# HBioquant/DiffBindFR

Hardware: AMD Instinct MI355X
Metric: poses_per_sec (higher is better)
Workload: dtype f32

## Files before the change

diffbindfr_amd/csrc/convz.hip:

```cpp
#include <cstdio>
#include <cstdlib>
#include <type_traits>

#include "common.h"

typedef float f32x4 __attribute__((ext_vector_type(4)));
typedef float f32x2 __attribute__((ext_vector_type(2)));
typedef _Float16 f16x8 __attribute__((ext_vector_type(8)));
typedef _Float16 f16x4 __attribute__((ext_vector_type(4)));
typedef _Float16 f16x2 __attribute__((ext_vector_type(2)));
typedef unsigned u32x4 __attribute__((ext_vector_type(4)));
typedef unsigned u32x2 __attribute__((ext_vector_type(2)));

#define CH_TILE_BYTES 9280
#define CH_TAIL_OFF 8192
#define CH_BIAS_OFF 9216

#define CZ_VSTRIDE 2064
#define CZ_CB (8 * CZ_VSTRIDE)
#define CZ_NCB 2
#define CZ_TILE (CZ_NCB * CZ_CB)
#define CZ_KPB 1
#define CZ_BUF (CZ_KPB * CZ_TILE)
#define CZ_ZBYTES (2 * CZ_BUF)
#define CZ_WAVE_FLOATS (32 * 12 + 32 + 32 + 32 + 32 + 32 + CZ_MAXSEG * 16 + 24 * 64)
#ifndef CZ_PRIO
#define CZ_PRIO 1
#endif
#if CZ_PRIO
#define CZ_SETPRIO(x) __builtin_amdgcn_s_setprio(x)
#else
#define CZ_SETPRIO(x)
#endif
#ifndef CZ_FETCH_AT
#define CZ_FETCH_AT 4
#endif
#ifndef CZ_PF_KT
#define CZ_PF_KT 7
#endif
#define CZ_ZSCALE (-20)

__device__ __forceinline__ void cz_split2(float x0, float x1, unsigned& hi, unsigned& lo) {
  const f16x2 h = __builtin_convertvector((f32x2){x0, x1}, f16x2);
  const f16x2 l = __builtin_convertvector((f32x2){x0 - (float)h[0], x1 - (float)h[1]}, f16x2);
  hi = __builtin_bit_cast(unsigned, h);
  lo = __builtin_bit_cast(unsigned, l);
}
__device__ __forceinline__ float cz_wave_max(float v) {
#pragma unroll
  for (int o = 1; o < 64; o <<= 1) v = fmaxf(v, __shfl_xor(v, o));
  return v;
}

template <int I, int N, typename F>
__device__ __forceinline__ void cz_static_for(F&& f) {
  if constexpr (I < N) { f(std::integral_constant<int, I>{}); cz_static_for<I + 1, N>(f); }
}

template <int NW, int ABL = 0>
__global__ __launch_bounds__(64 * NW, 2) void k_convz(ConvZArgs a) {
  constexpr int KT = 9;
  extern __shared__ __attribute__((aligned(16))) float lds[];
  const int tid = threadIdx.x, lane = tid & 63, wave = __builtin_amdgcn_readfirstlane(tid >> 6);
  const int n = lane & 15, g = lane >> 4;
  char* zb = reinterpret_cast<char*>(lds);
  float* wl = lds + CZ_ZBYTES / 4 + wave * CZ_WAVE_FLOATS;
  float* w_sh = wl;
  float* w_sa = wl + 32 * 12;
  float* w_ua = w_sa + 32;
  int* w_row = reinterpret_cast<int*>(w_ua + 32);
  int* w_seg = w_row + 32;
  int* w_first = w_seg + 32;
  unsigned* w_mask = reinterpret_cast<unsigned*>(w_first + 32);
  float* w_xs = reinterpret_cast<float*>(w_mask + CZ_MAXSEG * 16);
  int* b_nseg = reinterpret_cast<int*>(lds + CZ_ZBYTES / 4 + NW * CZ_WAVE_FLOATS);
  int* b_col_edge = b_nseg + NW;
  float* b_col_inv = reinterpret_cast<float*>(b_col_edge + 16 * CZ_NCB);
  unsigned* b_cdesc = reinterpret_cast<unsigned*>(b_col_inv + 16 * CZ_NCB);

  int tr_n = 0;
  auto stamp = [&](int tag) {
    if constexpr ((ABL & 128) != 0) {
      if (a.dbg && blockIdx.x == 0 && lane == 0 && tr_n < 1000) {
        unsigned long long* t = reinterpret_cast<unsigned long long*>(a.dbg) + wave * 1024;
        t[tr_n++] = (__builtin_amdgcn_s_memtime() << 8) | (unsigned)tag;
      }
    }
  };
  int nch[4] = {0, 0, 0, 0}, nu[4] = {0, 0, 0, 0};
#pragma unroll
  for (int c = 0; c < 4; ++c)
    if (c < a.n_conv) {
      const ConvZDesc& d = a.c[c];
      nch[c] = min(*d.n_chunks, d.max_chunks);
      nu[c] = (nch[c] + NW - 1) / NW;
    }
  const int N = nu[0] + nu[1] + nu[2] + nu[3];
  for (int unit = blockIdx.x; unit < N; unit += gridDim.x) {
    int c = 0, ul = unit;
    if (ul >= nu[0]) { ul -= nu[0]; c = 1; if (ul >= nu[1]) { ul -= nu[1]; c = 2; if (ul >= nu[2]) { ul -= nu[2]; c = 3; } } }
    const ConvZDesc& d = a.c[c];
    const ConvZ& W = d.w;
    const int E = min(*d.n_edges, d.max_edges);
    const int ch = ul * NW + wave;
    int es = 0, len = 0, gidx = 0;
    if (ch < nch[c]) {
      es = d.chunk_es[ch];
      const int gl = d.chunk_gl[ch];
      gidx = gl >> 6;
      len = min(min(gl & 63, 32), max(E - es, 0));
    }
    __syncthreads();
    if (tid < CZ_MAXCT * 16) b_cdesc[tid] = tid < (W.ct0[W.n_io - 1] + W.nct[W.n_io - 1]) * 16 ? W.cdesc[tid] : 0u;
    if (unit != (int)blockIdx.x) tr_n = 1000;
    stamp(1);
    const int sl = lane & 31;
    const bool have = len > 0;
    const int e_sl = have ? es + min(sl, len - 1) : 0;
    int tgt_l = 0, gth_l = 0;
    if (have) { tgt_l = d.tgt[e_sl]; gth_l = d.gth[e_sl]; }
    const int tgt_prev = __shfl_up(tgt_l, 1);
    const bool is_first = lane < 32 && sl < len && (sl == 0 || tgt_l != tgt_prev);
    const unsigned long long bal = __ballot(is_first);
    const unsigned firsts = (unsigned)bal;
    const int nseg = min(__popc(firsts), CZ_MAXSEG);
    const int seg_l = (sl < len) ? __popc(firsts & (0xffffffffu >> (31 - sl))) - 1 : -1;
    if (lane < 32) {
      w_row[sl] = gth_l * d.ldx;
      w_seg[sl] = seg_l;
      if (is_first) w_first[seg_l] = sl;
      const float* sp = d.sh + (size_t)e_sl * SH_LD;
#pragma unroll
      for (int k = 0; k < 9; ++k) w_sh[sl * 12 + k] = have ? sp[k] : 0.f;
      w_sh[sl * 12 + 9] = w_sh[sl * 12 + 10] = w_sh[sl * 12 + 11] = 0.f;
    }
    if (lane == 0) b_nseg[wave] = nseg;
    float xmx = 0.f, smx = 0.f;
    if (have) {
      if (d.xmax) xmx = d.xmax[gidx];
      else {
        const float* xr = d.x + (size_t)gth_l * d.ldx;
        const int d4 = d.ldx >> 2;
        for (int j = lane >> 5; j < d4; j += 2) {
          const f32x4 v = *reinterpret_cast<const f32x4*>(xr + 4 * j);
          xmx = fmaxf(fmaxf(xmx, fmaxf(fabsf(v[0]), fabsf(v[1]))), fmaxf(fabsf(v[2]), fabsf(v[3])));
        }
      }
      if (lane < 32) {
        const float* sp = d.sh + (size_t)e_sl * SH_LD;
#pragma unroll
        for (int k = 0; k < 9; ++k) smx = fmaxf(smx, fabsf(sp[k]));
      }
    }
    xmx = cz_wave_max(xmx); smx = cz_wave_max(smx);
    int ey = 0;
    if (xmx > 0.f && smx > 0.f) ey = max(-100, min(100, 13 - __builtin_amdgcn_frexp_expf(xmx) - __builtin_amdgcn_frexp_expf(smx)));
    ey = __builtin_amdgcn_readfirstlane(ey);
    const float sY = __builtin_amdgcn_ldexpf(1.f, ey);

    stamp(2);
    u32x4 Hh[CZ_NKT][2];
    int eh = 0;
    {
      const __amdgpu_buffer_rsrc_t rW1 = __builtin_amdgcn_make_buffer_rsrc((void*)W.W1h, 0, KT * CH_TILE_BYTES, 0x00020000);
      u32x4 Ah[2][2][4];
      u32x4 Atc[2];
#pragma unroll
      for (int et = 0; et < 2; ++et) {
        const int slot = 16 * et + n;
        const int e = have ? es + min(slot, len - 1) : 0;
        const float* r0 = d.emb + (size_t)e * NS;
        const float* r1 = d.tab1 + (size_t)(have ? d.idx1[e] : 0) * d.ld1;
        const float* r2 = d.tab2 + (size_t)(have ? d.idx2[e] : 0) * d.ld2;
        f32x4 Ba[KT];
        float amx = 0.f;
#pragma unroll
        for (int s4 = 0; s4 < KT; ++s4) {
          const float* src = s4 < 3 ? r0 : s4 < 6 ? r1 : r2;
          Ba[s4] = have ? *reinterpret_cast<const f32x4*>(src + 16 * (s4 % 3) + 4 * g) : (f32x4){0.f, 0.f, 0.f, 0.f};
#pragma unroll
          for (int q = 0; q < 4; ++q) amx = fmaxf(amx, fabsf(Ba[s4][q]));
        }
        amx = fmaxf(amx, __shfl_xor(amx, 16));
        amx = fmaxf(amx, __shfl_xor(amx, 32));
        const int ja = max(-14, __builtin_amdgcn_frexp_expf(amx));
        const float sa = __builtin_amdgcn_ldexpf(1.f, 15 - ja);
        if (g == 0) { w_sa[slot] = sa; w_ua[slot] = __builtin_amdgcn_ldexpf(1.f, ja - 15); }
#pragma unroll
        for (int s4 = 0; s4 < KT; ++s4) {
          unsigned hi0, lo0, hi1, lo1;
          cz_split2(Ba[s4][0] * sa, Ba[s4][1] * sa, hi0, lo0);
          cz_split2(Ba[s4][2] * sa, Ba[s4][3] * sa, hi1, lo1);
          if (s4 < 8) {
            Ah[et][0][s4 >> 1][2 * (s4 & 1)] = hi0; Ah[et][0][s4 >> 1][2 * (s4 & 1) + 1] = hi1;
            Ah[et][1][s4 >> 1][2 * (s4 & 1)] = lo0; Ah[et][1][s4 >> 1][2 * (s4 & 1) + 1] = lo1;
          } else {
            Atc[et] = (u32x4){lo0, lo1, hi0, hi1};
          }
        }
      }
      __builtin_amdgcn_wave_barrier();
      f32x4 sar[2], uar[2];
#pragma unroll
      for (int et = 0; et < 2; ++et) {
        sar[et] = *reinterpret_cast<const f32x4*>(w_sa + 16 * et + 4 * g);
        uar[et] = *reinterpret_cast<const f32x4*>(w_ua + 16 * et + 4 * g);
      }
      float Hf[KT][2][4];
      float hmx = 0.f;
      const int vW = lane * 16;
      u32x4 F[3][2];
      auto ldF = [&](auto ic) {
        constexpr int i = decltype(ic)::value, m = i / 5, sx = i % 5;
        if constexpr (sx < 4) {
          F[i % 3][0] = __builtin_bit_cast(u32x4, __builtin_amdgcn_raw_buffer_load_b128(rW1, vW, m * CH_TILE_BYTES + sx * 1024, 0));
          F[i % 3][1] = __builtin_bit_cast(u32x4, __builtin_amdgcn_raw_buffer_load_b128(rW1, vW, m * CH_TILE_BYTES + (4 + sx) * 1024, 0));
        } else {
          F[i % 3][0] = __builtin_bit_cast(u32x4, __builtin_amdgcn_raw_buffer_load_b128(rW1, vW, m * CH_TILE_BYTES + CH_TAIL_OFF, 0));
          F[i % 3][1][0] = __builtin_amdgcn_raw_buffer_load_b32(rW1, n * 4, m * CH_TILE_BYTES + CH_BIAS_OFF, 0);
        }
      };
      ldF(std::integral_constant<int, 0>{});
      ldF(std::integral_constant<int, 1>{});
      f32x4 acc[2];
      cz_static_for<0, 5 * KT>([&](auto ic) {
        constexpr int i = decltype(ic)::value, m = i / 5, sx = i % 5;
        if constexpr (i + 2 < 5 * KT) ldF(std::integral_constant<int, (i + 2 < 5 * KT ? i + 2 : 0)>{});
        if constexpr (sx == 0) { acc[0] = (f32x4){0.f, 0.f, 0.f, 0.f}; acc[1] = (f32x4){0.f, 0.f, 0.f, 0.f}; }
        if constexpr (sx < 4) {
          const f16x8 whi = __builtin_bit_cast(f16x8, F[i % 3][0]), wlo = __builtin_bit_cast(f16x8, F[i % 3][1]);
#pragma unroll
          for (int et = 0; et < 2; ++et) {
            acc[et] = __builtin_amdgcn_mfma_f32_16x16x32_f16(__builtin_bit_cast(f16x8, Ah[et][1][sx]), whi, acc[et], 0, 0, 0);
            acc[et] = __builtin_amdgcn_mfma_f32_16x16x32_f16(__builtin_bit_cast(f16x8, Ah[et][0][sx]), wlo, acc[et], 0, 0, 0);
            acc[et] = __builtin_amdgcn_mfma_f32_16x16x32_f16(__builtin_bit_cast(f16x8, Ah[et][0][sx]), whi, acc[et], 0, 0, 0);
          }
        } else {
          const u32x4 wt = F[i % 3][0];
          const f16x8 wf = __builtin_bit_cast(f16x8, wt);
          const f16x8 wh = __builtin_bit_cast(f16x8, (u32x4){wt[0], wt[1], 0u, 0u});
          const float bias = __builtin_bit_cast(float, F[i % 3][1][0]);
          const float w1r = W.W1rinv ? W.W1rinv[16 * m + n] : 1.f;
#pragma unroll
          for (int et = 0; et < 2; ++et) {
            acc[et] = __builtin_amdgcn_mfma_f32_16x16x32_f16(__builtin_bit_cast(f16x8, Atc[et]), wf, acc[et], 0, 0, 0);
            acc[et] = __builtin_amdgcn_mfma_f32_16x16x32_f16(__builtin_bit_cast(f16x8, (u32x4){Atc[et][2], Atc[et][3], 0u, 0u}), wh, acc[et], 0, 0, 0);
          }
#pragma unroll
          for (int et = 0; et < 2; ++et)
#pragma unroll
            for (int q = 0; q < 4; ++q) {
              const float v = fmaxf(acc[et][q] + bias * sar[et][q], 0.f) * (uar[et][q] * w1r);
              Hf[m][et][q] = v;
              hmx = fmaxf(hmx, v);
            }
        }
      });
      if (!(ABL & 128) && a.dbg && unit == 0 && wave == 0) {
        const float k1i = __builtin_amdgcn_ldexpf(1.f, -W.k1);
#pragma unroll
        for (int m = 0; m < KT; ++m)
#pragma unroll
          for (int et = 0; et < 2; ++et)
#pragma unroll
            for (int q = 0; q < 4; ++q) a.dbg[(16 * et + 4 * g + q) * 144 + 16 * m + n] = Hf[m][et][q] * k1i;
      }
      hmx = cz_wave_max(hmx);
      eh = max(hmx > 0.f ? __builtin_amdgcn_frexp_expf(hmx) : W.k1, W.k1);
      eh = min(eh, W.k1 + 100);
      const float sH = __builtin_amdgcn_ldexpf(1.f, 15 - eh);
#pragma unroll
      for (int m = 0; m < KT; ++m) {
        unsigned h0, l0, h1, l1, h2, l2, h3, l3;
        cz_split2(Hf[m][0][0] * sH, Hf[m][0][1] * sH, h0, l0);
        cz_split2(Hf[m][0][2] * sH, Hf[m][0][3] * sH, h1, l1);
        cz_split2(Hf[m][1][0] * sH, Hf[m][1][1] * sH, h2, l2);
        cz_split2(Hf[m][1][2] * sH, Hf[m][1][3] * sH, h3, l3);
        Hh[m][0] = (u32x4){h0, h1, h2, h3};
        Hh[m][1] = (u32x4){l0, l1, l2, l3};
      }
    }
    const int ephi = 15 - eh + W.k1;
    {
      const _Float16 ph = (_Float16)__builtin_amdgcn_ldexpf(1.f, ephi);
      const unsigned short pb = __builtin_bit_cast(unsigned short, ph);
      u32x4 hb = {0u, 0u, 0u, 0u};
      if (n == 0) {
#pragma unroll
        for (int t = 0; t < 8; ++t) {
          const int slot = t < 4 ? 4 * g + t : 16 + 4 * g + (t - 4);
          if (slot < len) hb[t >> 1] |= (unsigned)pb << (16 * (t & 1));
        }
      }
      Hh[KT][0] = hb;
      Hh[KT][1] = (u32x4){0u, 0u, 0u, 0u};
    }
    stamp(3);
    {
      const int j = lane >> 4, gg = (lane >> 2) & 3, r = lane & 3, t0 = 2 * r;
      const int s0 = t0 < 4 ? 4 * gg + t0 : 16 + 4 * gg + (t0 - 4);
      w_mask[lane] = (w_seg[s0] == j ? 0x0000ffffu : 0u) | (w_seg[s0 + 1] == j ? 0xffff0000u : 0u);
    }
    __builtin_amdgcn_wave_barrier();
    __syncthreads();
    int cbase = 0, total = 0;
#pragma unroll
    for (int v = 0; v < NW; ++v) { const int c = b_nseg[v]; if (v < wave) cbase += c; total += c; }
    cbase = __builtin_amdgcn_readfirstlane(cbase); total = __builtin_amdgcn_readfirstlane(total);
    const int nseg_u = __builtin_amdgcn_readfirstlane(nseg);
    const int ncb = (total + 15) >> 4;
    const float col_inv = __builtin_amdgcn_ldexpf(1.f, -CZ_ZSCALE - ey - ephi);
    const float zs = __builtin_amdgcn_ldexpf(1.f, CZ_ZSCALE);
    if (ABL & 32) continue;
    for (int c = tid; c < 16 * CZ_NCB; c += 64 * NW) b_col_edge[c] = -1;
    __syncthreads();
    if (lane < nseg_u) {
      b_col_edge[cbase + lane] = es + w_first[lane];
      b_col_inv[cbase + lane] = col_inv;
    }
    char* za[CZ_MAXSEG];
    {
      char* zw0 = zb + (n & 7) * CZ_VSTRIDE + g * 512 + (n >> 3) * 256;
#pragma unroll
      for (int j = 0; j < CZ_MAXSEG; ++j) {
        const int col = cbase + j;
        za[j] = j < nseg_u ? zw0 + (col >> 4) * CZ_CB + (col & 15) * 16 : zw0 + CZ_CB + 15 * 16;
      }
    }
    long long n_mfma = 2 * KT * 14;
    for (int io = 0; io < W.n_io; ++io) {
      n_mfma += (long long)W.nct[io] * (3LL * CZ_NKT * CZ_MAXSEG + 9LL * ncb * (KT + (wave == 0)));
      f32x4 acc[3][CZ_NCB];
#pragma unroll
      for (int wt = 0; wt < 3; ++wt)
#pragma unroll
        for (int cb = 0; cb < CZ_NCB; ++cb) acc[wt][cb] = (f32x4){0.f, 0.f, 0.f, 0.f};
      const char* wbase = reinterpret_cast<const char*>(W.W2z) + (size_t)lane * 16;
      int gq = W.ct0[io] * CZ_NKT;
      const int gq_last = (W.ct0[io] + W.nct[io]) * CZ_NKT - 1;
      u32x4 Wf[2][3][2];
      auto fetchW = [&](auto par_c, int q) {
        constexpr int par = decltype(par_c)::value;
        if ((ABL & 1) && q != W.ct0[io] * CZ_NKT) return;
        const char* p = wbase + ((size_t)q * 8 + wave) * CZ_TILE_BYTES;
#pragma unroll
        for (int wt = 0; wt < 3; ++wt)
#pragma unroll
          for (int pc = 0; pc < 2; ++pc) Wf[par][wt][pc] = *reinterpret_cast<const u32x4*>(p + (wt * 2 + pc) * 1024);
      };
      u32x4 Ym[CZ_MAXSEG][2];
#pragma unroll
      for (int j = 0; j < CZ_MAXSEG; ++j) { Ym[j][0] = (u32x4){0u, 0u, 0u, 0u}; Ym[j][1] = (u32x4){0u, 0u, 0u, 0u}; }
      auto prefetch_x = [&](int ct) {
        if (nseg_u == 0 || (ABL & 16)) return;
        const int lane = __builtin_amdgcn_mbcnt_hi(~0u, __builtin_amdgcn_mbcnt_lo(~0u, 0u)), n = lane & 15, g = lane >> 4;
        const unsigned cd_n = b_cdesc[(W.ct0[io] + ct) * 16 + n];
        const bool vec = (__builtin_amdgcn_readfirstlane(cd_n) >> 12) & 1u;
        const int xo = cd_n & 0xfff;
        const unsigned lds0 = (unsigned)(size_t)(const void __attribute__((address_space(3)))*)w_xs;
#pragma unroll
        for (int t = 0; t < 8; ++t) {
          const float* xp = d.x + w_row[t < 4 ? 4 * g + t : 16 + 4 * g + (t - 4)] + xo;
          asm volatile("s_mov_b32 m0, %0\n\ts_nop 0\n\tglobal_load_lds_dword %1, off" ::"s"(__builtin_amdgcn_readfirstlane(lds0 + t * 256)), "v"(xp) : "memory");
          if (vec) {
            asm volatile("s_mov_b32 m0, %0\n\ts_nop 0\n\tglobal_load_lds_dword %1, off" ::"s"(__builtin_amdgcn_readfirstlane(lds0 + (8 + t) * 256)), "v"(xp + 1) : "memory");
            asm volatile("s_mov_b32 m0, %0\n\ts_nop 0\n\tglobal_load_lds_dword %1, off" ::"s"(__builtin_amdgcn_readfirstlane(lds0 + (16 + t) * 256)), "v"(xp + 2) : "memory");
          }
        }
      };
      auto wait_stage = [&](auto younger_c) {
        constexpr int y = decltype(younger_c)::value;
        __builtin_amdgcn_sched_barrier(0);
        if constexpr (y == 0) asm volatile("s_waitcnt vmcnt(0)" ::: "memory");
        else asm volatile("s_waitcnt vmcnt(6)" ::: "memory");
        __builtin_amdgcn_sched_barrier(0);
      };
      auto finish_Y = [&](int ct) {
        if (nseg_u == 0 || (ABL & 16)) return;
        const int lane = __builtin_amdgcn_mbcnt_hi(~0u, __builtin_amdgcn_mbcnt_lo(~0u, 0u)), n = lane & 15, g = lane >> 4;
        const unsigned cd_n = b_cdesc[(W.ct0[io] + ct) * 16 + n];
        const bool vec = (__builtin_amdgcn_readfirstlane(cd_n) >> 12) & 1u;
        const int so = (cd_n >> 16) & 15;
        const float yv = (cd_n >> 31) ? sY : 0.f;
        float y[8];
        if (!vec) {
          float xs[8], s0[8];
#pragma unroll
          for (int t = 0; t < 8; ++t) { xs[t] = w_xs[t * 64 + lane]; s0[t] = w_sh[(t < 4 ? 4 * g + t : 16 + 4 * g + (t - 4)) * 12 + so]; }
#pragma unroll
          for (int t = 0; t < 8; ++t) y[t] = xs[t] * s0[t] * yv;
        } else {
          float xs[8][3], s1[8][3];
#pragma unroll
          for (int t = 0; t < 8; ++t)
#pragma unroll
            for (int m = 0; m < 3; ++m) { xs[t][m] = w_xs[(8 * m + t) * 64 + lane]; s1[t][m] = w_sh[(t < 4 ? 4 * g + t : 16 + 4 * g + (t - 4)) * 12 + so + m]; }
#pragma unroll
          for (int t = 0; t < 8; ++t) y[t] = (xs[t][0] * s1[t][0] + xs[t][1] * s1[t][1] + xs[t][2] * s1[t][2]) * yv;
        }
        u32x4 Yh, Yl;
#pragma unroll
        for (int r = 0; r < 4; ++r) { unsigned hi, lo; cz_split2(y[2 * r], y[2 * r + 1], hi, lo); Yh[r] = hi; Yl[r] = lo; }
#pragma unroll
        for (int j = 0; j < CZ_MAXSEG; ++j) {
          const u32x4 mk = *reinterpret_cast<const u32x4*>(w_mask + (j * 4 + g) * 4);
          Ym[j][0] = Yh & mk; Ym[j][1] = Yl & mk;
        }
      };
#define YM(j, p) __builtin_bit_cast(f16x8, Ym[j][p])
#define MF(a, b, c) __builtin_amdgcn_mfma_f32_16x16x32_f16(a, b, c, 0, 0, 0)
#define SL __builtin_amdgcn_sched_barrier(0)
      auto stepA = [&](auto kt_c, auto buf_c) {
        constexpr int kt = decltype(kt_c)::value, boff = decltype(buf_c)::value * CZ_BUF;
        if (ABL & 4) return;
        const f32x4 zero = {0.f, 0.f, 0.f, 0.f};
        const f16x8 hh = __builtin_bit_cast(f16x8, Hh[kt][0]), hl = __builtin_bit_cast(f16x8, Hh[kt][1]);
        f32x4 z[CZ_MAXSEG];
#pragma unroll
        for (int j = 0; j < CZ_MAXSEG; ++j) z[j] = MF(YM(j, 0), hl, zero);
#pragma unroll
        for (int j = 0; j < CZ_MAXSEG; ++j) z[j] = MF(YM(j, 1), hh, z[j]);
#pragma unroll
        for (int j = 0; j < CZ_MAXSEG; ++j) z[j] = MF(YM(j, 0), hh, z[j]);
#pragma unroll
        for (int j = 0; j < CZ_MAXSEG; ++j) *reinterpret_cast<f32x4*>(za[j] + boff) = z[j];
      };
      auto cut = [&](const f32x4 (&zf)[2], u32x4& zh, u32x4& zl, auto r_c) {
        constexpr int r = decltype(r_c)::value;
        unsigned hi, lo;
        cz_split2(zf[r >> 1][2 * (r & 1)] * zs, zf[r >> 1][2 * (r & 1) + 1] * zs, hi, lo);
        zh[r] = hi; zl[r] = lo;
      };
      using K0 = std::integral_constant<int, 0>; using K1 = std::integral_constant<int, 1>;
      using K2 = std::integral_constant<int, 2>; using K3 = std::integral_constant<int, 3>;
      auto tile = [&](auto kt_c, auto ncb_c) {
        constexpr int kt = decltype(kt_c)::value, NCBV = decltype(ncb_c)::value;
        constexpr int boffA = ((kt + 1) & 1) * CZ_BUF;
        if constexpr (CZ_FETCH_AT == 0) fetchW(std::integral_constant<int, (kt + 1) & 1>{}, min(gq + 1, gq_last));
        const char* zr = zb + (kt & 1) * CZ_BUF + wave * CZ_VSTRIDE + g * 512 + n * 16;
        f32x4 zf0[2], zf1[2];
        zf0[0] = *reinterpret_cast<const f32x4*>(zr); zf0[1] = *reinterpret_cast<const f32x4*>(zr + 256);
        const f32x4 zero = {0.f, 0.f, 0.f, 0.f};
        const f16x8 hh = __builtin_bit_cast(f16x8, Hh[kt + 1][0]), hl = __builtin_bit_cast(f16x8, Hh[kt + 1][1]);
        u32x4 p0h, p0l, p1h, p1l;
        f32x4 z0, z1, z2, z3;
        if constexpr ((ABL & 4) != 0) {
          z0 = z1 = z2 = z3 = zero;
          cut(zf0, p0h, p0l, K0{}); cut(zf0, p0h, p0l, K1{}); cut(zf0, p0h, p0l, K2{}); cut(zf0, p0h, p0l, K3{});
        } else {
        CZ_SETPRIO(3);
        SL;
        z0 = MF(YM(0, 0), hl, zero); SL;
        z1 = MF(YM(1, 0), hl, zero); SL;
        z2 = MF(YM(2, 0), hl, zero); SL;
        z3 = MF(YM(3, 0), hl, zero); SL;
        if constexpr (CZ_FETCH_AT == 4) { fetchW(std::integral_constant<int, (kt + 1) & 1>{}, min(gq + 1, gq_last)); SL; }
        z0 = MF(YM(0, 1), hh, z0); cut(zf0, p0h, p0l, K0{}); SL;
        z1 = MF(YM(1, 1), hh, z1); SL;
        z2 = MF(YM(2, 1), hh, z2); cut(zf0, p0h, p0l, K1{}); SL;
        z3 = MF(YM(3, 1), hh, z3); SL;
        if constexpr (CZ_FETCH_AT == 8) { fetchW(std::integral_constant<int, (kt + 1) & 1>{}, min(gq + 1, gq_last)); SL; }
        CZ_SETPRIO(2);
        z0 = MF(YM(0, 0), hh, z0); cut(zf0, p0h, p0l, K2{}); SL;
        z1 = MF(YM(1, 0), hh, z1); SL;
        z2 = MF(YM(2, 0), hh, z2); cut(zf0, p0h, p0l, K3{}); SL;
        z3 = MF(YM(3, 0), hh, z3); SL;
        if constexpr (CZ_FETCH_AT == 12) { fetchW(std::integral_constant<int, (kt + 1) & 1>{}, min(gq + 1, gq_last)); SL; }
        }
        if constexpr ((ABL & 4) != 0 && CZ_FETCH_AT != 0) fetchW(std::integral_constant<int, (kt + 1) & 1>{}, min(gq + 1, gq_last));
#define WFR(wt, pc) __builtin_bit_cast(f16x8, Wf[kt & 1][wt][pc])
        if constexpr ((ABL & 8) != 0) {
          if constexpr (!(ABL & 4)) { *reinterpret_cast<f32x4*>(za[0] + boffA) = z0; *reinterpret_cast<f32x4*>(za[1] + boffA) = z1; *reinterpret_cast<f32x4*>(za[2] + boffA) = z2; *reinterpret_cast<f32x4*>(za[3] + boffA) = z3; }
          asm volatile("" :: "v"(p0h), "v"(p0l));
        } else {
          const f16x8 zh = __builtin_bit_cast(f16x8, p0h), zl = __builtin_bit_cast(f16x8, p0l);
          if constexpr (NCBV > 1) { zf1[0] = *reinterpret_cast<const f32x4*>(zr + CZ_CB); zf1[1] = *reinterpret_cast<const f32x4*>(zr + CZ_CB + 256); }
          acc[0][0] = MF(WFR(0, 0), zl, acc[0][0]); *reinterpret_cast<f32x4*>(za[0] + boffA) = z0; SL;
          acc[1][0] = MF(WFR(1, 0), zl, acc[1][0]); *reinterpret_cast<f32x4*>(za[1] + boffA) = z1; SL;
          acc[2][0] = MF(WFR(2, 0), zl, acc[2][0]); *reinterpret_cast<f32x4*>(za[2] + boffA) = z2; SL;
          acc[0][0] = MF(WFR(0, 1), zh, acc[0][0]); *reinterpret_cast<f32x4*>(za[3] + boffA) = z3; SL;
          CZ_SETPRIO(1);
          acc[1][0] = MF(WFR(1, 1), zh, acc[1][0]); if constexpr (NCBV > 1) cut(zf1, p1h, p1l, K0{}); SL;
          acc[2][0] = MF(WFR(2, 1), zh, acc[2][0]); if constexpr (NCBV > 1) cut(zf1, p1h, p1l, K1{}); SL;
          acc[0][0] = MF(WFR(0, 0), zh, acc[0][0]); if constexpr (NCBV > 1) cut(zf1, p1h, p1l, K2{}); SL;
          acc[1][0] = MF(WFR(1, 0), zh, acc[1][0]); if constexpr (NCBV > 1) cut(zf1, p1h, p1l, K3{}); SL;
          acc[2][0] = MF(WFR(2, 0), zh, acc[2][0]); SL;
        }
        if constexpr (NCBV > 1 && !(ABL & 8)) {
          const f16x8 zh = __builtin_bit_cast(f16x8, p1h), zl = __builtin_bit_cast(f16x8, p1l);
          acc[0][1] = MF(WFR(0, 0), zl, acc[0][1]); SL;
          acc[1][1] = MF(WFR(1, 0), zl, acc[1][1]); SL;
          acc[2][1] = MF(WFR(2, 0), zl, acc[2][1]); SL;
          CZ_SETPRIO(0);
          acc[0][1] = MF(WFR(0, 1), zh, acc[0][1]); SL;
          acc[1][1] = MF(WFR(1, 1), zh, acc[1][1]); SL;
          acc[2][1] = MF(WFR(2, 1), zh, acc[2][1]); SL;
          acc[0][1] = MF(WFR(0, 0), zh, acc[0][1]); SL;
          acc[1][1] = MF(WFR(1, 0), zh, acc[1][1]); SL;
          acc[2][1] = MF(WFR(2, 0), zh, acc[2][1]); SL;
        }
      };
      auto tile9 = [&](int ct) {
        constexpr int kt = KT;
        wait_stage(K0{});
        if (wave == 0 && !(ABL & 8)) {
          const int lane = __builtin_amdgcn_mbcnt_hi(~0u, __builtin_amdgcn_mbcnt_lo(~0u, 0u)), n = lane & 15, g = lane >> 4;
          const char* zr = zb + (kt & 1) * CZ_BUF + g * 512 + n * 16;
#pragma unroll
          for (int cb = 0; cb < CZ_NCB; ++cb)
            if (cb < ncb) {
              f32x4 zf[2];
              zf[0] = *reinterpret_cast<const f32x4*>(zr + cb * CZ_CB); zf[1] = *reinterpret_cast<const f32x4*>(zr + cb * CZ_CB + 256);
              u32x4 ph, pl;
              cut(zf, ph, pl, K0{}); cut(zf, ph, pl, K1{}); cut(zf, ph, pl, K2{}); cut(zf, ph, pl, K3{});
              const f16x8 zh = __builtin_bit_cast(f16x8, ph), zl = __builtin_bit_cast(f16x8, pl);
#pragma unroll
              for (int wt = 0; wt < 3; ++wt) {
                acc[wt][cb] = MF(WFR(wt, 0), zl, acc[wt][cb]);
                acc[wt][cb] = MF(WFR(wt, 1), zh, acc[wt][cb]);
                acc[wt][cb] = MF(WFR(wt, 0), zh, acc[wt][cb]);
              }
            }
        }
        if (ct + 1 < W.nct[io]) { finish_Y(ct + 1); stepA(K0{}, K0{}); }
        __builtin_amdgcn_sched_barrier(0);
        fetchW(K0{}, min(gq + 1, gq_last));
      };
#undef WFR
      prefetch_x(0);
      wait_stage(K0{});
      fetchW(K0{}, gq);
      finish_Y(0);
      stepA(K0{}, K0{});
      __syncthreads();
      auto run_tiles = [&](auto ncb_c) {
        for (int ct = 0; ct < W.nct[io]; ++ct) {
          cz_static_for<0, CZ_NKT>([&](auto kt_c) {
            constexpr int kt = decltype(kt_c)::value;
            stamp(10);
            if constexpr (kt < KT) {
              tile(kt_c, ncb_c);
              if constexpr (kt == CZ_PF_KT) if (ct + 1 < W.nct[io]) prefetch_x(ct + 1);
            } else
              tile9(ct);
            stamp(12);
            ++gq;
            if (!(ABL & 2)) __syncthreads();
            stamp(13);
          });
        }
      };
      if (ncb > 1) run_tiles(K2{}); else run_tiles(K1{});
#undef YM
#undef MF
#undef SL
      float* red = reinterpret_cast<float*>(zb) + wave * (12 * CZ_NCB * 64);
#pragma unroll
      for (int wt = 0; wt < 3; ++wt)
#pragma unroll
        for (int cb = 0; cb < CZ_NCB; ++cb)
#pragma unroll
          for (int q = 0; q < 4; ++q) red[((wt * CZ_NCB + cb) * 4 + q) * 64 + lane] = acc[wt][cb][q];
      __syncthreads();
      for (int idx = tid; idx < 16 * ncb * 48; idx += 64 * NW) {
        const int col = idx / 48, w = idx - 48 * col;
        const int e = b_col_edge[col];
        if (e >= 0) {
          const int r = w & 15;
          const float* rp = reinterpret_cast<const float*>(zb) + (((w >> 4) * CZ_NCB + (col >> 4)) * 4 + (r & 3)) * 64 + 16 * (r >> 2) + (col & 15);
          float s = 0.f;
#pragma unroll
          for (int v = 0; v < NW; ++v) s += rp[v * (12 * CZ_NCB * 64)];
          d.msg[(size_t)e * d.D_out + W.out_off[io] + w] = s * b_col_inv[col] * W.rowinv[io * 48 + w];
        }
      }
      __syncthreads();
    }
    if (a.executed && lane == 0) atomicAdd(a.executed, 16384.0 * (double)n_mfma);
  }
}

__global__ void k_convz_useful(ConvZArgs a) {
  for (int c = 0; c < a.n_conv; ++c) {
    const ConvZDesc& d = a.c[c];
    const ConvZ& W = d.w;
    const int nch = min(*d.n_chunks, d.max_chunks), E = min(*d.n_edges, d.max_edges);
    double useful = 0.0, bytes = 0.0;
    for (int ch = blockIdx.x * blockDim.x + threadIdx.x; ch < nch; ch += gridDim.x * blockDim.x) {
      const int es = d.chunk_es[ch], len = min(min(d.chunk_gl[ch] & 63, 32), max(E - es, 0));
      int nseg = 0;
      for (int i = 0; i < len; ++i) nseg += (i == 0 || d.tgt[es + i] != d.tgt[es + i - 1]);
      nseg = min(nseg, CZ_MAXSEG);
      double u = 144.0 * 144.0 * len;
      for (int io = 0; io < W.n_io; ++io) u += (double)W.nc_valid[io] * 145.0 * ((double)len + 48.0 * nseg);
      useful += 6.0 * u;
      bytes += 4.0 * 48.0 * W.n_io * nseg;
    }
    if (useful > 0.0) { atomicAdd(a.executed + 1, useful); atomicAdd(a.executed + 2, bytes); }
  }
}

size_t convz_lds_bytes() { return CZ_ZBYTES + 8 * CZ_WAVE_FLOATS * sizeof(float) + (8 + 2 * 16 * CZ_NCB + CZ_MAXCT * 16) * sizeof(int); }

void launch_convz(const ConvZArgs& a0, hipStream_t st) {
  constexpr int NW = 8;
  ConvZArgs a = a0;
  static float* dbg_dev = nullptr;
  static const char* dbg_file = getenv("DBFR_CONVZ_DEBUG");
  if (dbg_file && !dbg_dev) {
    if (hipMalloc(&dbg_dev, 8 * 1024 * 8) != hipSuccess || hipMemset(dbg_dev, 0, 8 * 1024 * 8) != hipSuccess) dbg_dev = nullptr;
    else atexit([] {
      std::vector<float> h(8 * 1024 * 2);
      if (hipDeviceSynchronize() == hipSuccess && hipMemcpy(h.data(), dbg_dev, h.size() * 4, hipMemcpyDeviceToHost) == hipSuccess)
        if (FILE* f = fopen(getenv("DBFR_CONVZ_DEBUG"), "wb")) { fwrite(h.data(), 4, h.size(), f); fclose(f); }
    });
  }
  a.dbg = dbg_dev;
  const size_t lds = convz_lds_bytes();
#define V(x) { if (dbfr_launch_check(hipFuncSetAttribute(reinterpret_cast<const void*>(&k_convz<NW, x>), hipFuncAttributeMaxDynamicSharedMemorySize, (int)lds), "k_convz: hipFuncSetAttribute(MaxDynamicSharedMemorySize)")) return; \
               hipLaunchKernelGGL((k_convz<NW, x>), dim3(dbfr_current_cu_count()), dim3(64 * NW), lds, st, a); return; }
#ifdef DBFR_DEV_VARIANTS
  static int abl = getenv("DBFR_CONVZ_ABL") ? atoi(getenv("DBFR_CONVZ_ABL")) : 0;
  if (abl == 1) V(1) if (abl == 2) V(2) if (abl == 4) V(4) if (abl == 8) V(8) if (abl == 16) V(16) if (abl == 32) V(32) if (abl == 12) V(12) if (abl == 5) V(5) if (abl == 64) V(64) if (abl == 128) V(128)
#endif
  if (a.executed) hipLaunchKernelGGL(k_convz_useful, dim3(64), dim3(256), 0, st, a);
  V(0)
#undef V
}
```

Measured before the change: 494.2.

## Spill low-half H fragments to LDS and hoist next weight fetch in tile9

The low-precision halves of the first two H fragments are stored in per-wave LDS and reloaded when needed instead of held in registers, to relieve VGPR pressure. In tile9, the next weight tile is fetched before the wave-0 tail MFMAs, and the wait becomes vmcnt(6) so that fetch overlaps the tail compute instead of being issued after it. The fetch that precedes tile9 now reads wave 0's share, which is the weight slice tile9 uses. This adds LDS traffic and per-wave LDS footprint, and the reordered waitcnt relies on a fetch being exactly six loads.

```diff
diff --git a/diffbindfr_amd/csrc/convz.hip b/diffbindfr_amd/csrc/convz.hip
--- a/diffbindfr_amd/csrc/convz.hip
+++ b/diffbindfr_amd/csrc/convz.hip
@@ -23,7 +23,8 @@
 #define CZ_KPB 1
 #define CZ_BUF (CZ_KPB * CZ_TILE)
 #define CZ_ZBYTES (2 * CZ_BUF)
-#define CZ_WAVE_FLOATS (32 * 12 + 32 + 32 + 32 + 32 + 32 + CZ_MAXSEG * 16 + 24 * 64)
+#define CZ_NHL 2
+#define CZ_WAVE_FLOATS (32 * 12 + 32 + 32 + 32 + 32 + 32 + CZ_MAXSEG * 16 + 24 * 64 + CZ_NHL * 256)
 #ifndef CZ_PRIO
 #define CZ_PRIO 1
 #endif
@@ -50,6 +51,12 @@
 #pragma unroll
   for (int o = 1; o < 64; o <<= 1) v = fmaxf(v, __shfl_xor(v, o));
   return v;
+}
+
+__device__ __forceinline__ int cz_lane_here() {
+  int l = __builtin_amdgcn_mbcnt_hi(~0u, __builtin_amdgcn_mbcnt_lo(~0u, 0u));
+  asm volatile("" : "+v"(l));
+  return l;
 }
 
 template <int I, int N, typename F>
@@ -73,6 +80,7 @@
   int* w_first = w_seg + 32;
   unsigned* w_mask = reinterpret_cast<unsigned*>(w_first + 32);
   float* w_xs = reinterpret_cast<float*>(w_mask + CZ_MAXSEG * 16);
+  u32x4* w_hl = reinterpret_cast<u32x4*>(w_xs + 24 * 64);
   int* b_nseg = reinterpret_cast<int*>(lds + CZ_ZBYTES / 4 + NW * CZ_WAVE_FLOATS);
   int* b_col_edge = b_nseg + NW;
   float* b_col_inv = reinterpret_cast<float*>(b_col_edge + 16 * CZ_NCB);
@@ -277,7 +285,8 @@
         cz_split2(Hf[m][1][0] * sH, Hf[m][1][1] * sH, h2, l2);
         cz_split2(Hf[m][1][2] * sH, Hf[m][1][3] * sH, h3, l3);
         Hh[m][0] = (u32x4){h0, h1, h2, h3};
-        Hh[m][1] = (u32x4){l0, l1, l2, l3};
+        if (m < CZ_NHL) w_hl[m * 64 + lane] = (u32x4){l0, l1, l2, l3};
+        else Hh[m][1] = (u32x4){l0, l1, l2, l3};
       }
     }
     const int ephi = 15 - eh + W.k1;
@@ -339,10 +348,10 @@
       int gq = W.ct0[io] * CZ_NKT;
       const int gq_last = (W.ct0[io] + W.nct[io]) * CZ_NKT - 1;
       u32x4 Wf[2][3][2];
-      auto fetchW = [&](auto par_c, int q) {
+      auto fetchW = [&](auto par_c, int q, int share) {
         constexpr int par = decltype(par_c)::value;
         if ((ABL & 1) && q != W.ct0[io] * CZ_NKT) return;
-        const char* p = wbase + ((size_t)q * 8 + wave) * CZ_TILE_BYTES;
+        const char* p = wbase + ((size_t)q * 8 + share) * CZ_TILE_BYTES;
 #pragma unroll
         for (int wt = 0; wt < 3; ++wt)
 #pragma unroll
@@ -370,6 +379,7 @@
       };
       auto wait_stage = [&](auto younger_c) {
         constexpr int y = decltype(younger_c)::value;
+        static_assert(y == 0 || y == 6, "wait_stage: a fetch is six loads");
         __builtin_amdgcn_sched_barrier(0);
         if constexpr (y == 0) asm volatile("s_waitcnt vmcnt(0)" ::: "memory");
         else asm volatile("s_waitcnt vmcnt(6)" ::: "memory");
@@ -377,7 +387,7 @@
       };
       auto finish_Y = [&](int ct) {
         if (nseg_u == 0 || (ABL & 16)) return;
-        const int lane = __builtin_amdgcn_mbcnt_hi(~0u, __builtin_amdgcn_mbcnt_lo(~0u, 0u)), n = lane & 15, g = lane >> 4;
+        const int lane = cz_lane_here(), n = lane & 15, g = lane >> 4;
         const unsigned cd_n = b_cdesc[(W.ct0[io] + ct) * 16 + n];
         const bool vec = (__builtin_amdgcn_readfirstlane(cd_n) >> 12) & 1u;
         const int so = (cd_n >> 16) & 15;
@@ -410,11 +420,18 @@
 #define YM(j, p) __builtin_bit_cast(f16x8, Ym[j][p])
 #define MF(a, b, c) __builtin_amdgcn_mfma_f32_16x16x32_f16(a, b, c, 0, 0, 0)
 #define SL __builtin_amdgcn_sched_barrier(0)
+      auto load_hl = [&](auto kt_c) -> u32x4 {
+        constexpr int kt = decltype(kt_c)::value;
+        if constexpr (kt < CZ_NHL) {
+          return w_hl[kt * 64 + cz_lane_here()];
+        } else
+          return Hh[kt][1];
+      };
       auto stepA = [&](auto kt_c, auto buf_c) {
         constexpr int kt = decltype(kt_c)::value, boff = decltype(buf_c)::value * CZ_BUF;
         if (ABL & 4) return;
         const f32x4 zero = {0.f, 0.f, 0.f, 0.f};
-        const f16x8 hh = __builtin_bit_cast(f16x8, Hh[kt][0]), hl = __builtin_bit_cast(f16x8, Hh[kt][1]);
+        const f16x8 hh = __builtin_bit_cast(f16x8, Hh[kt][0]), hl = __builtin_bit_cast(f16x8, load_hl(kt_c));
         f32x4 z[CZ_MAXSEG];
 #pragma unroll
         for (int j = 0; j < CZ_MAXSEG; ++j) z[j] = MF(YM(j, 0), hl, zero);
@@ -436,12 +453,12 @@
       auto tile = [&](auto kt_c, auto ncb_c) {
         constexpr int kt = decltype(kt_c)::value, NCBV = decltype(ncb_c)::value;
         constexpr int boffA = ((kt + 1) & 1) * CZ_BUF;
-        if constexpr (CZ_FETCH_AT == 0) fetchW(std::integral_constant<int, (kt + 1) & 1>{}, min(gq + 1, gq_last));
+        if constexpr (CZ_FETCH_AT == 0) fetchW(std::integral_constant<int, (kt + 1) & 1>{}, min(gq + 1, gq_last), kt + 1 == KT ? 0 : wave);
         const char* zr = zb + (kt & 1) * CZ_BUF + wave * CZ_VSTRIDE + g * 512 + n * 16;
         f32x4 zf0[2], zf1[2];
         zf0[0] = *reinterpret_cast<const f32x4*>(zr); zf0[1] = *reinterpret_cast<const f32x4*>(zr + 256);
         const f32x4 zero = {0.f, 0.f, 0.f, 0.f};
-        const f16x8 hh = __builtin_bit_cast(f16x8, Hh[kt + 1][0]), hl = __builtin_bit_cast(f16x8, Hh[kt + 1][1]);
+        const f16x8 hh = __builtin_bit_cast(f16x8, Hh[kt + 1][0]), hl = __builtin_bit_cast(f16x8, load_hl(std::integral_constant<int, kt + 1>{}));
         u32x4 p0h, p0l, p1h, p1l;
         f32x4 z0, z1, z2, z3;
         if constexpr ((ABL & 4) != 0) {
@@ -454,20 +471,20 @@
         z1 = MF(YM(1, 0), hl, zero); SL;
         z2 = MF(YM(2, 0), hl, zero); SL;
         z3 = MF(YM(3, 0), hl, zero); SL;
-        if constexpr (CZ_FETCH_AT == 4) { fetchW(std::integral_constant<int, (kt + 1) & 1>{}, min(gq + 1, gq_last)); SL; }
+        if constexpr (CZ_FETCH_AT == 4) { fetchW(std::integral_constant<int, (kt + 1) & 1>{}, min(gq + 1, gq_last), kt + 1 == KT ? 0 : wave); SL; }
         z0 = MF(YM(0, 1), hh, z0); cut(zf0, p0h, p0l, K0{}); SL;
         z1 = MF(YM(1, 1), hh, z1); SL;
         z2 = MF(YM(2, 1), hh, z2); cut(zf0, p0h, p0l, K1{}); SL;
         z3 = MF(YM(3, 1), hh, z3); SL;
-        if constexpr (CZ_FETCH_AT == 8) { fetchW(std::integral_constant<int, (kt + 1) & 1>{}, min(gq + 1, gq_last)); SL; }
+        if constexpr (CZ_FETCH_AT == 8) { fetchW(std::integral_constant<int, (kt + 1) & 1>{}, min(gq + 1, gq_last), kt + 1 == KT ? 0 : wave); SL; }
         CZ_SETPRIO(2);
         z0 = MF(YM(0, 0), hh, z0); cut(zf0, p0h, p0l, K2{}); SL;
         z1 = MF(YM(1, 0), hh, z1); SL;
         z2 = MF(YM(2, 0), hh, z2); cut(zf0, p0h, p0l, K3{}); SL;
         z3 = MF(YM(3, 0), hh, z3); SL;
-        if constexpr (CZ_FETCH_AT == 12) { fetchW(std::integral_constant<int, (kt + 1) & 1>{}, min(gq + 1, gq_last)); SL; }
-        }
-        if constexpr ((ABL & 4) != 0 && CZ_FETCH_AT != 0) fetchW(std::integral_constant<int, (kt + 1) & 1>{}, min(gq + 1, gq_last));
+        if constexpr (CZ_FETCH_AT == 12) { fetchW(std::integral_constant<int, (kt + 1) & 1>{}, min(gq + 1, gq_last), kt + 1 == KT ? 0 : wave); SL; }
+        }
+        if constexpr ((ABL & 4) != 0 && CZ_FETCH_AT != 0) fetchW(std::integral_constant<int, (kt + 1) & 1>{}, min(gq + 1, gq_last), kt + 1 == KT ? 0 : wave);
 #define WFR(wt, pc) __builtin_bit_cast(f16x8, Wf[kt & 1][wt][pc])
         if constexpr ((ABL & 8) != 0) {
           if constexpr (!(ABL & 4)) { *reinterpret_cast<f32x4*>(za[0] + boffA) = z0; *reinterpret_cast<f32x4*>(za[1] + boffA) = z1; *reinterpret_cast<f32x4*>(za[2] + boffA) = z2; *reinterpret_cast<f32x4*>(za[3] + boffA) = z3; }
@@ -502,9 +519,10 @@
       };
       auto tile9 = [&](int ct) {
         constexpr int kt = KT;
-        wait_stage(K0{});
+        fetchW(K0{}, min(gq + 1, gq_last), wave);
+        wait_stage(std::integral_constant<int, 6>{});
         if (wave == 0 && !(ABL & 8)) {
-          const int lane = __builtin_amdgcn_mbcnt_hi(~0u, __builtin_amdgcn_mbcnt_lo(~0u, 0u)), n = lane & 15, g = lane >> 4;
+          const int lane = cz_lane_here(), n = lane & 15, g = lane >> 4;
           const char* zr = zb + (kt & 1) * CZ_BUF + g * 512 + n * 16;
 #pragma unroll
           for (int cb = 0; cb < CZ_NCB; ++cb)
@@ -523,17 +541,15 @@
             }
         }
         if (ct + 1 < W.nct[io]) { finish_Y(ct + 1); stepA(K0{}, K0{}); }
-        __builtin_amdgcn_sched_barrier(0);
-        fetchW(K0{}, min(gq + 1, gq_last));
       };
 #undef WFR
       prefetch_x(0);
       wait_stage(K0{});
-      fetchW(K0{}, gq);
-      finish_Y(0);
-      stepA(K0{}, K0{});
-      __syncthreads();
       auto run_tiles = [&](auto ncb_c) {
+        fetchW(K0{}, gq, wave);
+        finish_Y(0);
+        stepA(K0{}, K0{});
+        __syncthreads();
         for (int ct = 0; ct < W.nct[io]; ++ct) {
           cz_static_for<0, CZ_NKT>([&](auto kt_c) {
             constexpr int kt = decltype(kt_c)::value;
```

New measurement: 518.5 (median of 6 runs). 1.05x the previous value.
